# oma219/spumoni

Hardware: AMD Instinct MI355X
Metric: reads/s PML classification, 200 bp reads vs 10-hap human index (higher is better)
Workload: dtype u64

## Files before the change

### spumoni_amd/capi.py

```python
from __future__ import annotations

import ctypes as C
import os
import subprocess
from typing import Optional

import numpy as np

_HERE = os.path.dirname(os.path.abspath(__file__))
LIB_PATH = os.environ.get("SPUMONI_GPU_LIB") or os.path.join(_HERE, "libspumoni_gpu.so")
CSRC = os.path.join(_HERE, "csrc")

SPX_MODE_PML = 0
SPX_MODE_MS = 1

EXPORTS = [
    "spx_last_error",
    "spx_device_count",
    "spx_index_from_runs",
    "spx_index_load_raw",
    "spx_index_free",
    "spx_index_stats",
    "spx_index_device_bytes",
    "spx_index_set_text",
# ... 349 lines not shown
        st = stream if stream is not None else torch.cuda.current_stream(self.device)
        nreads = d_offs.numel() - 1
        cap = int(lib().spx_digest_capacity(kind, k, total_chars))
        if work is None or work[0].numel() < cap or work[1].numel() < nreads + 1:
            work = (torch.empty(cap, dtype=torch.uint8, device=d_seqs.device),
                    torch.empty(nreads + 1, dtype=torch.int64, device=d_seqs.device))
        narrow = any(t is not None and t.element_size() == 2 for t in (d_lengths, d_docs))
        fn = lib().spx_digest_query_batch_device16 if narrow else lib().spx_digest_query_batch_device
        _check(fn(self._h, mode, kind, k, w, _t_ptr(d_seqs), _t_ptr(d_offs), nreads, total_chars, _t_ptr(work[0]), work[0].numel(),
                  _t_ptr(work[1]), _t_ptr(d_lengths), _t_ptr(d_pointers), _t_ptr(d_docs), _t_ptr(d_class), bin_width, max_value_thr,
                  C.c_void_p(st.cuda_stream)))
        return work[1], work

    def digest_query_host(self, mode, kind, k, w, seqs, offs, want_lengths=True, want_docs=False, classify=None):
        seqs = np.ascontiguousarray(seqs, dtype=np.uint8)
        offs = np.ascontiguousarray(offs, dtype=np.uint64)
        nreads = offs.size - 1
        tot = int(offs[-1]) if nreads > 0 else 0
        cap = int(lib().spx_digest_capacity(kind, k, tot))
        out_offs = np.zeros(nreads + 1, dtype=np.uint64)
        lens = np.zeros(cap, dtype=np.uint32) if want_lengths else None
        ptrs = np.zeros(cap, dtype=np.uint64) if mode == SPX_MODE_MS else None
        docs = np.zeros(cap, dtype=np.uint32) if want_docs else None
        cls_ = np.zeros(max(nreads, 1), dtype=CLASS_DTYPE) if classify else None
        bw, thr = classify if classify else (0, 0)
        _check(lib().spx_digest_query_batch(self._h, mode, kind, k, w, _np_ptr(seqs), _np_ptr(offs), nreads,
                                            _np_ptr(out_offs), cap, _np_ptr(lens), _np_ptr(ptrs), _np_ptr(docs),
                                            _np_ptr(cls_), bw, thr))
        dt = int(out_offs[-1])
        out = {"offsets": out_offs}
        if lens is not None:
            out["lengths"] = lens[:dt]
        if ptrs is not None:
            out["pointers"] = ptrs[:dt]
        if docs is not None:
            out["docs"] = docs[:dt]
        if cls_ is not None:
            out["class"] = cls_[:nreads]
        return out

    def votes_device(self, d_lengths, d_docs, d_offs, min_length, d_out=None, stream=None):
        import torch

        L = _spv()
        st = stream if stream is not None else torch.cuda.current_stream(self.device)
        nreads = d_offs.numel() - 1
        if d_lengths.element_size() != d_docs.element_size():
            raise SpxError("d_lengths and d_docs must have the same width")
        if d_out is None:
            d_out = torch.empty((max(nreads, 0), 4), dtype=torch.int32, device=d_offs.device)
        _check(L.spv_votes_device(self._h, _t_ptr(d_lengths), _t_ptr(d_docs), d_lengths.element_size() * 8, _t_ptr(d_offs),
                                  nreads, min(d_lengths.numel(), d_docs.numel()), int(min_length), _t_ptr(d_out),
                                  C.c_void_p(st.cuda_stream)))
        return d_out

    def assign_host(self, mode, seqs, offs, min_length, digest=None):
        from .docvote import VOTE_DTYPE

        L = _spv()
        seqs = np.ascontiguousarray(seqs, dtype=np.uint8)
        offs = np.ascontiguousarray(offs, dtype=np.uint64)
        nreads = offs.size - 1
        kind, k, w = digest if digest else (0, 0, 0)
        rec = np.zeros(max(nreads, 1), dtype=VOTE_DTYPE)
        vals = np.zeros(max(nreads, 1), dtype=np.uint64)
        _check(L.spv_assign_batch(self._h, mode, kind, k, w, _np_ptr(seqs), _np_ptr(offs), nreads, int(min_length),
                                  _np_ptr(rec), _np_ptr(vals)))
        out = np.zeros(nreads, dtype=np.dtype(VOTE_DTYPE.descr + [("values", "<u8")]))
        for f in VOTE_DTYPE.names:
            out[f] = rec[f][:nreads]
        out["values"] = vals[:nreads]
        return out

    def votes_stats(self) -> dict:
        s = SpvVotesStats()
        _check(_spv().spv_last_votes_stats(self._h, C.byref(s)))
        return {f[0]: getattr(s, f[0]) for f in SpvVotesStats._fields_}

    def last_chunk_stats(self) -> dict:
        o = (C.c_uint64 * 4)()
        _check(lib().spx_last_chunk_stats(self._h, C.byref(o)))
        return {"chunk_len": o[0], "chunks_bound": o[1], "rewalked_chars": o[2], "fallback_reads": o[3]}

    def last_stats(self) -> dict:
        s = SpxWalkStats()
        _check(lib().spx_last_walk_stats(self._h, C.byref(s)))
        return {f[0]: getattr(s, f[0]) for f in SpxWalkStats._fields_}


def digester(device: int = 0) -> "Index":
    import torch

    from .synth import RawIndex

    z = torch.zeros(1, dtype=torch.int64)
    return Index.from_raw(RawIndex(heads=torch.zeros(1, dtype=torch.uint8), lens=torch.ones(1, dtype=torch.int64),
                                   thr=z, n=1), device)


def pinned_array(shape, dtype):
    n = int(np.prod(shape)) * np.dtype(dtype).itemsize
    p = lib().spx_host_alloc(max(n, 1))
    if not p:
        raise SpxError(lib().spx_last_error().decode())
    buf = (C.c_char * max(n, 1)).from_address(p)
    arr = np.frombuffer(buf, dtype=dtype, count=int(np.prod(shape))).reshape(shape)

    free = lib().spx_host_free

    class _Owner:
        def __del__(self_inner):
            try:
                free(p)
            except Exception:
                pass

    return arr, _Owner()


def pad_seqs(seqs):
    import torch

    n = seqs.numel()
    padded = torch.zeros(((n + 3) // 4) * 4 + 32, dtype=torch.uint8, device=seqs.device)
    padded[:n] = seqs
    return padded


DOCVOTE_EXPORTS = ["spv_votes_device", "spv_assign_batch", "spv_last_votes_stats"]
_SPV_READY = False


class SpvVotesStats(C.Structure):
    _fields_ = [("reads_short", C.c_uint64), ("reads_medium", C.c_uint64), ("reads_long", C.c_uint64),
                ("reads_empty", C.c_uint64), ("voting_positions", C.c_uint64), ("long_tiles", C.c_uint64),
                ("kernel_ms", C.c_float)]


def _spv() -> C.CDLL:
    global _SPV_READY
    L = lib()
    if not hasattr(L, "spv_assign_batch"):
        raise SpxError(f"{LIB_PATH} has no document votes (spv_assign_batch): there is no CPU fallback")
    if not _SPV_READY:
        vp, u64, u32, i32 = C.c_void_p, C.c_uint64, C.c_uint32, C.c_int
        L.spv_votes_device.argtypes = [vp, vp, vp, i32, vp, u64, u64, u64, vp, vp]
        L.spv_assign_batch.argtypes = [vp, i32, i32, u32, u32, vp, vp, u64, u64, vp, vp]
        L.spv_last_votes_stats.argtypes = [vp, C.POINTER(SpvVotesStats)]
        _SPV_READY = True
    return L


_SPB_READY = False


def _spb() -> C.CDLL:
    global _SPB_READY
    L = lib()
    if not hasattr(L, "spb_build_from_text"):
        raise SpxError(f"{LIB_PATH} has no index builder (spb_build_from_text): there is no CPU fallback for the HIP path")
    if not _SPB_READY:
        vp, u64 = C.c_void_p, C.c_uint64
        L.spb_build_from_text.restype = vp
        L.spb_build_from_text.argtypes = [vp, u64, vp, C.c_uint32, C.c_int, C.c_int]
        L.spb_build_stats.argtypes = [vp, C.POINTER(u64), C.POINTER(u64)]
        L.spb_build_copy.argtypes = [vp, vp, vp, vp, vp, vp, vp, vp]
# ... 85 lines not shown
```

### spumoni_amd/csrc/spx_internal.h

```cpp
#pragma once
#include <hip/hip_runtime.h>

#include <memory>
#include <functional>
#include <mutex>
#include <string>

#include "../../include/spumoni_gpu.h"
#include "spx_layout.h"

namespace spx {

void set_error(const char* fmt, ...);
int hip_fail(hipError_t e, const char* what, const char* file, int line);
int select_device(int device);

#define SPX_HIP(call)                                                        \
    do {                                                                     \
        hipError_t e_ = (call);                                              \
        if (e_ != hipSuccess) return spx::hip_fail(e_, #call, __FILE__, __LINE__); \
    } while (0)

struct QuietOnError {
    hipStream_t st;
    bool device_wide;
    bool ok = false;
    explicit QuietOnError(hipStream_t s, bool wide = false) : st(s), device_wide(wide) {}
    int done(int rc) {
        ok = rc == SPX_OK;
        return rc;
    }
    ~QuietOnError() {
        if (ok) return;
        if (device_wide)
            (void)hipDeviceSynchronize();
        else
            (void)hipStreamSynchronize(st);
    }
};

struct WalkCounters {
    unsigned long long reserved0;
    unsigned long long steps;
    unsigned long long jumps;
    unsigned long long pred_jumps;
    unsigned long long row_loads;
    unsigned long long dir_loads;
    unsigned long long error;
    unsigned long long pad_;
    unsigned long long claim;
};

struct ChunkDesc {
    uint64_t gend;
    uint32_t len;
    uint32_t rd;
};
struct WalkState {
    uint32_t k0;
    uint32_t length;
    uint64_t offp;
    uint64_t sample;
    uint32_t doc;
    uint32_t flags;
};
struct SeamRec {
    uint64_t t;
    uint32_t met;
    uint32_t reset_above;
    WalkState ext;
    uint32_t spec_length, spec_doc;
    uint64_t spec_sample;
};
constexpr uint32_t CKPT_SHIFT = 4;

struct ChunkArgs {
    const ChunkDesc* desc;
    const uint64_t* nchunks;
    WalkState* ends;
    WalkState* ckpt;
    SeamRec* seams;
    uint8_t* flags;
    uint32_t* read_fail;
    const uint64_t* chunk_start;
    WalkState* reentry;
    uint64_t* vtop;
    uint32_t* pending;
    uint32_t round;
    uint32_t last_round;
};
constexpr uint32_t CHUNK_TOP = 0x80000000u, CHUNK_BOTTOM = 0x40000000u, CHUNK_ACTIVE = 0x20000000u;
constexpr uint32_t CHUNK_LEN_MASK = 0x1fffffffu;
constexpr int CHUNK_EXTRA_ROUNDS = 3;

struct BatchArgs {
    const uint8_t* seqs;
    const uint64_t* offs;
    uint64_t nreads;
    uint64_t total_chars;
    uint32_t* out_lengths;
    uint64_t* out_pointers;
    uint32_t* out_docs;
    spx_class* out_class;
    uint64_t bin_width;
    uint64_t bin_magic;
    uint64_t max_value_thr;
    WalkCounters* counters;
    uint32_t lanes_per_wave;
    uint32_t narrow;
    ChunkArgs ch;
    const uint32_t* only_flagged;
    const uint64_t* in_starts;
    uint64_t* len_mask;
    unsigned long long* claim;
    uint64_t len_mask_pairs;
};

}

namespace spx {
struct ArrayOwner {
    int device = 0;
    void* p[10] = {};
    ~ArrayOwner() {
        (void)hipSetDevice(device);
        for (void* a : p)
            if (a) (void)hipFree(a);
    }
};
}

struct spx_index {
    int device = 0;
// ... 147 lines not shown
```

### spumoni_amd/csrc/spx_query.hip

```cpp
#include <algorithm>
#include <chrono>
#include <cstdio>
#include <cstring>
#include <thread>

#include "spx_internal.h"

using namespace spx;

extern "C" {

struct PubSrc {
    const uint64_t* one[4];
    const uint64_t* more;
    int nmore;
};
__global__ void k_publish(uint64_t* dst, PubSrc src) {
    const int t = (int)threadIdx.x;
    if (t < 4) dst[t] = src.one[t] ? *src.one[t] : 0;
    if (t >= 4 && t - 4 < src.nmore) dst[t] = src.more[t - 4];
    __threadfence_system();
}
static int publish(spx_index* ix, const PubSrc& src, hipStream_t st) {
    if (!ix->h_pub) {
        SPX_HIP(hipHostMalloc((void**)&ix->h_pub, 64 * sizeof(uint64_t), hipHostMallocMapped | hipHostMallocCoherent));
        SPX_HIP(hipHostGetDevicePointer((void**)&ix->h_pub_dev, ix->h_pub, 0));
    }
    k_publish<<<1, 64, 0, st>>>(ix->h_pub_dev, src);
    SPX_HIP(hipGetLastError());
    return SPX_OK;
}

uint64_t spx_digest_capacity(int kind, uint32_t k, uint64_t total_chars) {
    const uint64_t body = (kind == SPX_DIGEST_DNA ? (uint64_t)(k ? k : 1) : 1ull) * total_chars;
    return ((body + 3) / 4) * 4 + 32;
}

int spx_digest_batch_device(spx_index* ix, int kind, uint32_t k, uint32_t w, const uint8_t* d_seqs,
                            const uint64_t* d_offsets, uint64_t nreads, uint64_t total_chars,
                            uint8_t* d_out_seqs, uint64_t out_capacity, uint64_t* d_out_offsets, void* stream) {
    if (!ix || !d_seqs || !d_offsets || !d_out_seqs || !d_out_offsets) {
        set_error("null argument");
        return SPX_E_ARG;
    }
    if (((uintptr_t)d_seqs & 15) != 0) {
        set_error("d_seqs must be 16-byte aligned (and readable for round_up(total_chars, 16) + 16 bytes)");
        return SPX_E_ARG;
    }
    if (out_capacity < spx_digest_capacity(kind, k, total_chars)) {
        set_error("d_out_seqs must hold spx_digest_capacity() = %llu bytes",
                  (unsigned long long)spx_digest_capacity(kind, k, total_chars));
        return SPX_E_ARG;
    }
    std::lock_guard<std::mutex> g(ix->mu);
    SPX_HIP(hipSetDevice(ix->device));
    hipStream_t st = (hipStream_t)stream;
    return launch_digest(ix, kind, k, w, d_seqs, d_offsets, nreads, total_chars, d_out_seqs, d_out_offsets, st);
}

static int digest_for_walk(spx_index* ix, int mode, bool ms_lengths, int kind, uint32_t k, uint32_t w, const uint8_t* d_raw,
                           const uint64_t* d_offs, uint64_t nreads, uint64_t total_in, uint8_t* d_dig, uint64_t cap,
                           uint64_t* d_dig_offs, void* stream, const uint64_t** in_starts) {
    *in_starts = nullptr;
    if (!ix || !d_raw || !d_offs || !d_dig || !d_dig_offs) {
        set_error("null argument");
        return SPX_E_ARG;
    }
    if (((uintptr_t)d_raw & 15) != 0) {
        set_error("d_seqs must be 16-byte aligned (and readable for round_up(total_chars, 16) + 16 bytes)");
        return SPX_E_ARG;
    }
    if (cap < spx_digest_capacity(kind, k, total_in)) {
        set_error("the buffer for the digested reads must hold spx_digest_capacity() = %llu bytes",
                  (unsigned long long)spx_digest_capacity(kind, k, total_in));
        return SPX_E_ARG;
    }
    static const bool old_walk = getenv("SPX_OLD_WALK") != nullptr;
    static const int env_parked = getenv("SPX_DIGEST_PARKED") ? atoi(getenv("SPX_DIGEST_PARKED")) : -1;
    const int parked_mode = env_parked >= 0 ? env_parked : ix->digest_parked;
    std::lock_guard<std::mutex> g(ix->mu);
    SPX_HIP(hipSetDevice(ix->device));
    if (ix->num_cus == 0) {
        hipDeviceProp_t prop;
        SPX_HIP(hipGetDeviceProperties(&prop, ix->device));
        ix->num_cus = prop.multiProcessorCount;
    }
    bool park = parked_mode != 1 && ix->rows != nullptr && ix->view.compact && !old_walk && nreads > 0 && nreads < (1ull << 31) &&
                !(mode == SPX_MODE_MS && ms_lengths) && ix->force_lanes_per_wave == 0 &&
                (parked_mode == 2 || nreads * 2 > (uint64_t)ix->num_cus * 20 * 64);
// ... 676 lines not shown
        (void)hipEventRecord(fe[0], st);
    }
    const double t0 = std::chrono::duration<double>(std::chrono::steady_clock::now().time_since_epoch()).count();
    for (int i = 0; i < 3; ++i) {
        if (ix->text_bytes[i] == 0) continue;
        if (text[i]) SPX_HIP(hipMemcpyAsync(text[i], ix->scratch[spx_index::S_TEXT + i].p, ix->text_bytes[i], hipMemcpyDeviceToHost, st));
        if (line_start && line_start[i])
            SPX_HIP(hipMemcpyAsync(line_start[i], ix->scratch[spx_index::S_LINE_START + i].p, (ix->text_nreads + 1) * 8, hipMemcpyDeviceToHost, st));
    }
    if (ix->text_cls_host)
        SPX_HIP(hipMemcpyAsync(ix->text_cls_host, ix->scratch[spx_index::S_CLASS].p, ix->text_nreads * sizeof(spx_class), hipMemcpyDeviceToHost, st));
    if (phase_trace) (void)hipEventRecord(fe[1], st);
    if ((rc = ctx_wait(ix, st)) != SPX_OK) return rc;
    if (phase_trace) {
        float a = 0;
        (void)hipEventElapsedTime(&a, fe[0], fe[1]);
        fprintf(stderr, "[phases] %p fetch: copy out %.3f ms (behind the digits' kernels)\n", (void*)ix, a);
    }
    ix->text_cls_host = nullptr;
    ix->text_ready = false;
    if (timing)
        fprintf(stderr, "[spx] text_fetch: %.2f ms for %.1f MB\n",
                (std::chrono::duration<double>(std::chrono::steady_clock::now().time_since_epoch()).count() - t0) * 1e3,
                (ix->text_bytes[0] + ix->text_bytes[1] + ix->text_bytes[2]) / 1e6);
    return SPX_OK;
}

int spx_query_text_reserve(spx_index* ix, int mode, int digest_kind, uint32_t k, uint64_t max_chars, uint64_t max_reads,
                           uint32_t streams, int with_class, const uint64_t text_bytes[3]) {
    if (!ix || (mode != SPX_MODE_PML && mode != SPX_MODE_MS)) {
        set_error("spx_query_text_reserve: index and a mode");
        return SPX_E_ARG;
    }
    std::lock_guard<std::mutex> hg(ix->host_mu);
    std::lock_guard<std::mutex> g(ix->mu);
    SPX_HIP(hipSetDevice(ix->device));
    hipStream_t st = nullptr;
    int rc;
    if ((rc = ctx_stream_of(ix, &st)) != SPX_OK) return rc;
    const ScratchPlan plan = text_plan(mode, digest_kind, k, max_chars, max_chars, max_reads, streams, with_class != 0, text_bytes, true);
    void* p = nullptr;
    for (int i = 0; i < plan.n; ++i)
        if ((rc = ix->scratch[plan.item[i].slot].reserve(plan.item[i].bytes, &p)) != SPX_OK) return rc;
    const bool need_len = (streams & SPX_TEXT_LENGTHS) || (mode == SPX_MODE_MS && with_class);
    if (mode == SPX_MODE_PML && need_len &&
        (rc = ix->chunk_scr[spx_index::C_LEN_BITS].reserve(len_mask_pairs(max_chars, max_reads) * 16, &p)) != SPX_OK)
        return rc;
    if (!ix->h_pub) {
        PubSrc none{{nullptr, nullptr, nullptr, nullptr}, nullptr, 0};
        if ((rc = publish(ix, none, st)) != SPX_OK) return rc;
    }
    SPX_HIP(hipStreamSynchronize(st));
    return SPX_OK;
}

static int last_counters(spx_index* ix, bool after_ev1, WalkCounters& wc) {
    if (!ix->have_timing) {
        set_error("no query has run on this index yet");
        return SPX_E_ARG;
    }
    SPX_HIP(hipSetDevice(ix->device));
    if (after_ev1) SPX_HIP(hipEventSynchronize(ix->ev1));
    SPX_HIP(hipStreamSynchronize(ix->last_stream));
    SPX_HIP(hipMemcpy(&wc, ix->counters, sizeof wc, hipMemcpyDeviceToHost));
    return SPX_OK;
}

int spx_last_chunk_stats(spx_index* ix, uint64_t out[4]) {
    if (!ix || !out) {
        set_error("null argument");
        return SPX_E_ARG;
    }
    std::lock_guard<std::mutex> g(ix->mu);
    WalkCounters wc;
    const int rc = last_counters(ix, false, wc);
    if (rc != SPX_OK) return rc;
    out[0] = ix->last_chunk_len;
    out[1] = ix->last_chunk_bound;
    out[2] = wc.reserved0;
    out[3] = wc.pad_;
    return SPX_OK;
}

int spx_last_walk_stats(spx_index* ix, spx_walk_stats* out) {
    if (!ix || !out) {
        set_error("null argument");
        return SPX_E_ARG;
    }
    std::lock_guard<std::mutex> g(ix->mu);
    WalkCounters wc;
    const int rc = last_counters(ix, true, wc);
    if (rc != SPX_OK) return rc;
    float ms = 0;
    SPX_HIP(hipEventElapsedTime(&ms, ix->ev0, ix->ev1));
    out->steps = wc.steps;
    out->jumps = wc.jumps;
    out->pred_jumps = wc.pred_jumps;
    out->row_loads = wc.row_loads;
    out->dir_loads = wc.dir_loads;
    out->kernel_ms = ms;
    return walk_error(wc, WALK_ERR_STATS);
}

}
```

### spumoni_amd/csrc/spx_walk_fast.inc

```

enum : uint32_t { Q_LAND = 0, Q_FAT = 1, Q_STEP = 2, Q_READ = 3, Q_CHARS = 4, Q_FATJ = 5, Q_QS = 6, Q_DIR = 7, Q_DONE = 8, Q_SAMP = 9, Q_START = 10, Q_WANT = 11 };
enum : uint32_t {
    F_EMB = 1,
    F_NOROW = 2,
    F_QUIRK = 4,
    F_WIDE = 16,
    F_FADD = 32,
    F_HAVEC = 64,
    F_SAMPD = 128
};
enum : uint32_t { A_STEP = 1, A_EMIT = 2, A_DECIDE = 4 };
#ifndef SPX_STEP_REPS
#define SPX_STEP_REPS 2
#endif
constexpr int STEP_REPS = SPX_STEP_REPS;
constexpr uint32_t OFF_LAST32 = 0xffffffffu;
#ifndef SPX_CHUNK_CLAIM
#define SPX_CHUNK_CLAIM 64
#endif
constexpr uint32_t CHUNK_CLAIM = SPX_CHUNK_CLAIM;
static_assert(CHUNK_CLAIM >= 64, "a claim covers at least one iteration's worst case: 64 lanes ending a read each");

__device__ __forceinline__ uint32_t dpp_swap1(uint32_t v) { return (uint32_t)__builtin_amdgcn_mov_dpp((int)v, 0xB1, 0xf, 0xf, true); }

struct alignas(16) HotLetter {
    uint32_t bmul;
    uint32_t present;
    uint64_t fat0;
};

__device__ __forceinline__ void lf_target_ct(uint32_t LFrun, uint32_t LFoff, uint32_t cums, uint32_t off, uint32_t& k0,
                                             uint32_t& offp, uint32_t& t_out) {
    lf_target_c(LFrun, LFoff, cums, off, k0, offp);
    const uint32_t t = k0 - LFrun;
    t_out = (t < 4 && off <= 126) ? t : 4u;
}

template <int MODE, bool DOC, bool NARROW, int CHUNK = 0, bool EARLY = false, bool DYN = false>
__global__ void __launch_bounds__(WALK_TPB) k_walk_fast(const DevIndex ix, const BatchArgs b) {
    constexpr bool AUX = (MODE == SPX_MODE_MS) || DOC;
    constexpr bool PML = MODE == SPX_MODE_PML;
    if (CHUNK == 2 && b.ch.round > 1 && b.ch.pending[b.ch.round] == 0) return;
    __shared__ HotLetter s_hot[256];
#ifndef SPX_PGRP
#define SPX_PGRP 16
#endif
    constexpr int PGRP = SPX_PGRP, PROW = WALK_TPB + 1;
    constexpr int PLPG = PGRP / 2, PNG = 64 / PLPG;
    __shared__ uint64_t s_ptrs[MODE == SPX_MODE_MS && CHUNK != 2 ? PGRP * PROW : 1];
    constexpr bool DSTAGE = PML && DOC && CHUNK != 2;
    constexpr int DGRP = 32, DROW = DGRP + 2;
    __shared__ uint16_t s_docs[DSTAGE ? WALK_TPB * DROW : 1];
    const LetterInfo* const s_let = ix.letters;
    __shared__ uint32_t s_win[8 * WALK_TPB];
    const char* const rows_b = reinterpret_cast<const char*>(ix.rows);
    const char* const fat_b = reinterpret_cast<const char*>(ix.fat);
    const uint32_t fs = ix.fat_stride;
    const bool lrow = !AUX && fs == 32 && ix.aux == nullptr;
    for (int t = threadIdx.x; t < 256; t += blockDim.x) {
        const LetterInfo li = ix.letters[t];
        s_hot[t] = HotLetter{li.bmul, li.qbeg != li.qend ? 1u : 0u, (uint64_t)(uintptr_t)(fat_b + li.fbase * fs)};
    }
    __syncthreads();
    const char* const dir_b = reinterpret_cast<const char*>(ix.dirrows);
    const char* const fatj_b = reinterpret_cast<const char*>(ix.fat_js);
    const char* const q_b = reinterpret_cast<const char*>(ix.Q);
    const char* const seq_b = reinterpret_cast<const char*>(b.seqs);
    const char* const off_b = reinterpret_cast<const char*>(b.offs);
    const uint32_t R = ix.r;
    const uint32_t fs_shift = fs == 32 ? 5 : 4;
    const bool want_class = PML && CHUNK == 0 && b.out_class != nullptr;
    const bool want_len = PML && CHUNK != 2 && b.out_lengths != nullptr;
    const uint32_t lpw = b.lanes_per_wave;
    const uint32_t nlanes = (uint32_t)((((uint64_t)gridDim.x * blockDim.x) >> 6) * lpw);
    const uint32_t nitems = CHUNK ? (uint32_t)*b.ch.nchunks : (uint32_t)b.nreads;
    const uint64_t ch_org = CHUNK ? b.offs[0] : 0;
    uint8_t* const ch_flags = CHUNK ? b.ch.flags - (ch_org & ~7ull) : nullptr;
    WalkState* const ch_ckpt = CHUNK ? b.ch.ckpt - (ch_org >> CKPT_SHIFT) : nullptr;
    const char* const item_b = CHUNK ? reinterpret_cast<const char*>(b.ch.desc) : off_b;
    constexpr uint32_t ITEM_BYTES = CHUNK ? sizeof(ChunkDesc) : 8;
    const uint32_t tid = threadIdx.x;
    static_assert(!DYN || (CHUNK == 0 && !EARLY), "only the plain, full launch deals its reads on demand");
    uint32_t w_n0 = 0, w_e0 = 0, w_n1 = 0, w_e1 = 0;
    bool w_pend = false;
    bool w_dry = false;
    uint32_t w_wait = DYN ? (uint32_t)((((uint64_t)blockIdx.x * blockDim.x + tid) >> 6) & 31u) + 1u : 0u;
    unsigned long long claimed = 0;

    uint32_t rd = (uint32_t)((((uint64_t)blockIdx.x * blockDim.x + tid) >> 6) * lpw) + (tid & 63);
    uint32_t ph = (rd < nitems && (tid & 63) < lpw) ? Q_READ : Q_DONE;
    const char* addr = ph == Q_READ ? item_b + (uint64_t)rd * ITEM_BYTES : item_b;
    uint32_t seen = 0;
    uint64_t fb = 0;
    uint32_t fl = 0;
    uint32_t c = 0;
    uint64_t base = 0, ibase = 0;
    uint32_t m = 0, x = 0;
    int32_t wi = -1;
    uint64_t q0 = 0, q1 = 0;
    uint32_t k = 0, off = 0;
    uint32_t length = 0;
    uint64_t mbits = 0;
    uint32_t nr = 0;
    uint32_t bin_lo = 0, bin_max = 0, above = 0, below = 0;
    uint64_t sum_max = 0;
    uint64_t sample = 0;
    uint32_t doc = 0;
    uint32_t w_jumps = 0, w_pred = 0, w_rows = 0, w_dir = 0, w_again = 0;
    uint32_t tlimit = 0xffffffffu;
    V16 cka{0, 0, 0, 0}, ckb{0, 0, 0, 0};

#define WIN_AT(w) ((s_win[((uint32_t)(w) >> 2) * WALK_TPB + tid] >> (((uint32_t)(w) & 3) * 8)) & 0xffu)
#define CUR_C c
#define COUNT(var, cond) (var += (uint32_t)__popcll(__builtin_amdgcn_ballot_w64(cond)))

    V16 ga{0, 0, 0, 0}, gb{0, 0, 0, 0};
    uint32_t side_doc = 0;
    Aux side_aux{0, 0};
    uint64_t side_in = 0;
    auto issue_gather = [&]() {
        ga = V16{0, 0, 0, 0};
        gb = V16{0, 0, 0, 0};
#ifndef SPX_PAIR_MIN
#define SPX_PAIR_MIN 24
#endif
        constexpr int pair_min = EARLY ? 65 : SPX_PAIR_MIN;
        if ((int)__popcll(__builtin_amdgcn_ballot_w64(ph != Q_DONE && (fl & F_WIDE))) < pair_min) {
            if (ph != Q_DONE) {
                ga = *reinterpret_cast<const V16*>(addr);
                if (fl & F_WIDE) gb = *reinterpret_cast<const V16*>(addr + 16);
            }
        } else
        {
            typedef uint32_t u32x4 __attribute__((ext_vector_type(4), aligned(4)));
            typedef const __attribute__((address_space(1))) u32x4* GV16;
            const bool odd = tid & 1;
            const bool live = ph != Q_DONE;
            const uint32_t w_own = (live && (fl & F_WIDE)) ? 16u : 0u;
            const uint64_t au = (uint64_t)(uintptr_t)(live ? addr : rows_b);
            const uint64_t pu = u64of(dpp_swap1((uint32_t)au), dpp_swap1((uint32_t)(au >> 32))) + 16;
            const uint32_t w_for = dpp_swap1(w_own);
            const uint64_t a1 = odd ? pu : au, a2 = odd ? au : pu;
            const bool do1 = odd ? w_for != 0 : live, do2 = odd ? live : w_for != 0;
            uint32_t r1x = 0, r1y = 0, r1z = 0, r1w = 0, r2x = 0, r2y = 0, r2z = 0, r2w = 0;
            if (do1) {
                const u32x4 t = *(GV16)(uintptr_t)a1;
                r1x = t.x, r1y = t.y, r1z = t.z, r1w = t.w;
            }
            if (do2) {
                const u32x4 t = *(GV16)(uintptr_t)a2;
                r2x = t.x, r2y = t.y, r2z = t.z, r2w = t.w;
            }
            ga = V16{odd ? r2x : r1x, odd ? r2y : r1y, odd ? r2z : r1z, odd ? r2w : r1w};
            const uint32_t zx = dpp_swap1(odd ? r1x : r2x), zy = dpp_swap1(odd ? r1y : r2y), zz = dpp_swap1(odd ? r1z : r2z),
                           zw = dpp_swap1(odd ? r1w : r2w);
            gb = V16{w_own ? zx : 0u, w_own ? zy : 0u, w_own ? zz : 0u, w_own ? zw : 0u};
        }
        side_doc = 0;
        side_aux = Aux{0, 0};
        side_in = 0;
        claimed = 0;
        if (CHUNK == 0 && b.in_starts != nullptr && ph == Q_READ) side_in = b.in_starts[rd];
        if (DOC && ph == Q_SAMP) side_doc = ix.rundocs[k];
        if (AUX && ph == Q_DIR) side_aux = ix.aux[length];
        if (DYN && w_pend && (tid & 63) == 0) claimed = atomicAdd(b.claim, (unsigned long long)CHUNK_CLAIM);
    };
    if (EARLY) issue_gather();
    while (__builtin_amdgcn_ballot_w64(ph != Q_DONE) != 0) {
        if (!EARLY) issue_gather();
        uint32_t act = 0, hd = 0;
        uint32_t rflag = 0;
        bool pred_ev = false;
        uint32_t d_trun = 0, d_toff = 0, d_srun = 0, d_soff = 0, d_bits = 0;
        Aux d_aux{0, 0};
        bool d_lrow = false;
        uint64_t fbits = 0;
        uint32_t fxi = 0;
        bool flush = false;
        bool pflush = false, pheld = false, pheld_end = false;
        uint32_t pfxi = 0;
        uint64_t phold = 0;
        COUNT(w_rows, ph == Q_LAND);
        COUNT(w_dir, ph == Q_FAT || (ph >= Q_FATJ && ph <= Q_DIR));

        if (ph == Q_LAND) {
            const uint32_t len = ga.x & 0xffffu;
            const uint32_t o = off == OFF_LAST32 ? len - 1 : off;
            if (o >= len) {
                off = o - len;
                k++;
                addr += sizeof(Row32);
            } else {
                off = o;
                q0 = u64of(ga.x, ga.y);
                q1 = u64of(ga.z, ga.w);
                fl = (fl & ~F_NOROW) | F_EMB;
                act = A_STEP;
            }
        } else if (ph == Q_FAT) {
            const uint32_t hq = ga.x;
            const uint32_t w1l = ga.z, w1h = ga.w;
            const bool nosucc = (w1h >> 29) & 1, esc = (w1h >> 30) & 1;
            const bool quirk = fl & F_QUIRK;
            const bool found = nosucc || hq > k || (quirk && hq == k);
            if (found && !esc && !quirk) {
                d_trun = hq - (w1l & 0x7ffffu);
                d_toff = ((w1l >> 20) | (w1h << 12)) & 0xffffu;
                d_srun = ga.y;
                const uint32_t sfield = (w1h >> 4) & 0xffffu;
                const bool ps = (w1h >> 28) & 1;
                d_soff = ps ? sfield : 0u;
                d_bits = ((w1h >> 20) & 0xffu) | ((uint32_t)ps << 8) | ((uint32_t)nosucc << 9) | ((w1h >> 31) << 10) |
                         ((ps ? 0u : (sfield & 0xffu)) << 16);
                if (AUX) d_aux = Aux{u64of(gb.x, gb.y), u64of(gb.z, gb.w)};
                d_lrow = lrow;
                act = A_DECIDE;
            } else if (!found && (w1l & (uint32_t)FAT_SINGLE) && !(fl & F_FADD)) {
                fl |= F_FADD;
                addr += fs;
            } else if (found && esc && !quirk) {
                length = ga.y;
                fl |= F_WIDE;
                ph = Q_DIR;
                addr = dir_b + (uint64_t)length * sizeof(JumpRow);
            } else {
                const uint64_t grp = ((uint64_t)(addr - fat_b) >> fs_shift) >> FJ_SHIFT;
                length = (uint32_t)grp & 3;
                fl &= ~F_WIDE;
                ph = Q_FATJ;
                addr = fatj_b + ((grp * 4) & ~15ull);
            }
        } else if (ph == Q_STEP) {
            act = A_STEP;
        } else if (ph != Q_DONE && ph != Q_SAMP && (!DYN || ph != Q_WANT)) {
            if (ph == Q_READ) {
                if (CHUNK) {
                    m = ga.z & CHUNK_LEN_MASK;
                    base = u64of(ga.x, ga.y) - m;
                    seen = 0;
                    fb = 0;
                    if (CHUNK == 2 && (((ga.z >> 29) & 4) || (b.ch.round > 1 && !((ga.z >> 29) & 1)))) m = 0;
                } else {
                    base = u64of(ga.x, ga.y);
                    m = (uint32_t)(u64of(ga.z, ga.w) - base);
                }
                ibase = (CHUNK == 0 && b.in_starts != nullptr) ? side_in : base;
                if (m == 0) {
                    if (want_class) b.out_class[rd] = spx_class{0, 0, 0};
                    rd += DYN ? 0u : nlanes;
                    ph = DYN ? Q_WANT : (rd < nitems ? Q_READ : Q_DONE);
                    addr = DYN ? rows_b : item_b + (uint64_t)rd * ITEM_BYTES;
                } else {
                    if (NARROW && CHUNK == 0 && m >= 65536) atomicAdd(&b.counters->error, 1ull);
                    x = m;
                    length = 0;
                    sample = ix.init_sample;
                    doc = ix.init_doc;
                    k = ix.init_k;
                    off = (uint32_t)ix.init_off;
                    q0 = ix.init_row.q0;
                    q1 = ix.init_row.q1;
                    fl = 0;
                    wi = -1;
                    mbits = 0;
                    nr = m;
                    if (want_class) {
                        const uint32_t w = (uint32_t)b.bin_width;
                        const uint32_t q = w > 1 ? (uint32_t)__umul64hi((uint64_t)m, b.bin_magic) : m;
                        const uint32_t nb = q > 0 ? q : 1;
                        bin_lo = (nb - 1) * w;
                        bin_max = above = below = 0;
                        sum_max = 0;
                    }
                    act = A_STEP;
                    if (CHUNK == 2) {
                        ph = Q_START;
                        addr = reinterpret_cast<const char*>(b.ch.round > 1 ? b.ch.reentry + rd : b.ch.ends + rd + 1);
                        fl = F_WIDE;
                        act = 0;
                    }
                }
            } else if (ph == Q_CHARS) {
                s_win[0 * WALK_TPB + tid] = ga.x;
                s_win[1 * WALK_TPB + tid] = ga.y;
                s_win[2 * WALK_TPB + tid] = ga.z;
                s_win[3 * WALK_TPB + tid] = ga.w;
                s_win[4 * WALK_TPB + tid] = gb.x;
                s_win[5 * WALK_TPB + tid] = gb.y;
                s_win[6 * WALK_TPB + tid] = gb.z;
                s_win[7 * WALK_TPB + tid] = gb.w;
                ph = Q_STEP;
                act = A_STEP;
            } else if (CHUNK == 2 && ph == Q_START) {
                k = ga.x;
                length = ga.y;
                {
                    const uint64_t offp = u64of(ga.z, ga.w);
                    off = offp == OFF_END ? OFF_LAST32 : (uint32_t)offp;
                }
                sample = u64of(gb.x, gb.y);
                doc = gb.z;
                tlimit = b.ch.round > 1 ? gb.w : 0xffffffffu;
                ph = Q_LAND;
                addr = rows_b + (uint64_t)k * sizeof(Row32);
                fl = F_WIDE;
                {
                    const char* const cp = reinterpret_cast<const char*>(ch_ckpt + ((base + m - 1) >> CKPT_SHIFT));
                    cka = *reinterpret_cast<const V16*>(cp);
                    ckb = *reinterpret_cast<const V16*>(cp + 16);
                }
            } else if (ph == Q_FATJ) {
                const uint32_t lo = (length & 2) ? ga.z : ga.x, hi = (length & 2) ? ga.w : ga.y;
                length = (length & 1) ? hi : lo;
                fl |= F_WIDE;
                ph = Q_QS;
                addr = q_b + (uint64_t)length * 4;
            } else if (ph == Q_QS) {
                const uint32_t e[8] = {ga.x, ga.y, ga.z, ga.w, gb.x, gb.y, gb.z, gb.w};
                const uint32_t room_q = s_let[CUR_C].qend - length;
                uint32_t skip = 0;
#pragma unroll
                for (int t = 0; t < 8; ++t) skip += ((uint32_t)t < room_q && e[t] < k) ? 1u : 0u;
                length += skip;
                if (skip < 8) {
                    ph = Q_DIR;
                    addr = dir_b + (uint64_t)length * sizeof(JumpRow);
                } else {
                    addr = q_b + (uint64_t)length * 4;
                }
            } else {
                JumpRow e;
                e.d0 = u64of(ga.x, ga.y);
                e.d1 = u64of(ga.z, ga.w);
                e.d2 = u64of(gb.x, gb.y);
                e.d3 = u64of(gb.z, gb.w);
                const uint32_t jdir = length;
                const uint32_t qbeg = s_let[CUR_C].qbeg, qend = s_let[CUR_C].qend;
                if (!(fl & F_QUIRK)) {
                    d_trun = jr_THRrun(e);
                    d_toff = (uint32_t)jr_THRoff(e);
                    d_srun = jr_sLFrun(e);
                    d_soff = (uint32_t)jr_sLFoff(e);
                    d_bits = jr_Hs(e) | ((uint32_t)jr_psame(e) << 8) | ((jdir < qend ? 0u : 1u) << 9) | ((jdir <= qbeg ? 1u : 0u) << 10);
                    if (AUX) d_aux = side_aux;
                    act = A_DECIDE;
                } else {
                    const bool has_succ = jdir < qend;
                    const uint32_t trun = jr_THRrun(e);
                    const bool below_thr = !has_succ || (k < trun) || (k == trun && off < (uint32_t)jr_THRoff(e));
                    const uint32_t LFrun_k = (uint32_t)(q0 >> 32), LFoff_k = (uint32_t)(q0 >> 16) & 0xffffu;
                    pred_ev = below_thr;
                    if (AUX) {
                        const Aux a = ix.aux[jdir + ((below_thr && off > 0) ? 1u : 0u)];
                        if (MODE == SPX_MODE_MS) sample = below_thr ? aux_se(a) : aux_ss(a);
                        if (DOC) doc = below_thr ? (aux_docs(a) >> 16) : (aux_docs(a) & 0xffffu);
                    }
                    if (!below_thr) {
                        k = LFrun_k;
                        off = LFoff_k + off;
                    } else if (off > 0) {
                        k = LFrun_k;
                        off = LFoff_k + off - 1;
                    } else {
                        if (jdir <= qbeg) atomicAdd(&b.counters->error, 1ull);
                        const bool ps = jr_psame(e);
                        const uint32_t srun = jr_sLFrun(e);
                        k = ps ? srun : srun - 1;
                        off = ps ? (uint32_t)jr_sLFoff(e) - 1 : OFF_LAST32;
                    }
                    length = 0;
                    fl &= ~(F_EMB | F_QUIRK);
                    rflag = 3;
                    act = A_EMIT;
                }
            }
        }
        if (AUX && ph == Q_SAMP) {
            if (MODE == SPX_MODE_MS) sample = u64of(ga.x, ga.y);
            if (DOC) doc = side_doc & 0xffffu;
            fl |= F_SAMPD;
            ph = Q_STEP;
            act = A_STEP;
        }

        {
            const bool dec = act & A_DECIDE;
            const bool nosucc = (d_bits >> 9) & 1, psame = (d_bits >> 8) & 1;
            const bool below_thr = nosucc || (k < d_trun) || (k == d_trun && off < d_toff);
            COUNT(w_pred, (dec && below_thr) || pred_ev);
            if (dec) {
                if (below_thr && ((d_bits >> 10) & 1)) atomicAdd(&b.counters->error, 1ull);
                const bool last = below_thr && !psame;
                k = d_srun - (last ? 1u : 0u);
                off = last ? OFF_LAST32 : d_soff - (below_thr ? 1u : 0u);
                hd = last ? ((d_bits >> 16) & 0xffu) : (d_bits & 0xffu);
                if (MODE == SPX_MODE_MS) sample = below_thr ? aux_se(d_aux) : aux_ss(d_aux);
                if (DOC) doc = below_thr ? (aux_docs(d_aux) >> 16) : (aux_docs(d_aux) & 0xffffu);
                length = 0;
                fl = (fl & ~(F_EMB | F_QUIRK)) | ((d_lrow && !last) ? F_EMB : 0u);
                rflag = 3;
                act = A_EMIT;
            }
        }

#pragma unroll
        for (int rep = 0; rep < STEP_REPS; ++rep) {
            if (rep > 0 && __builtin_amdgcn_ballot_w64(act != 0) == 0) break;
            bool jumped = false;
            if (act & A_STEP) {
                const bool havec = fl & F_HAVEC;
                if (!havec && wi < 0) {
                    const uint64_t g = ibase + x - 1;
                    const uint64_t end4 = (g + 4) & ~3ull;
                    const uint64_t wbase = end4 >= 32 ? end4 - 32 : 0;
                    wi = (int32_t)(g - wbase);
                    ph = Q_CHARS;
                    addr = seq_b + wbase;
                    fl = (fl | F_WIDE) & ~F_EMB;
                    act = 0;
                } else {
                    const uint32_t cw = WIN_AT(wi < 0 ? 0 : wi);
                    c = havec ? c : cw;
                    wi -= havec ? 0 : 1;
                    const HotLetter hl = s_hot[c];
                    const uint32_t H = (uint32_t)q1 & 0xffu;
                    const bool eq = k < R && H == c;
                    const bool lf = eq && (c < 128 || ((q1 >> 8) & 1));
                    const bool present = hl.present != 0;
                    const bool go_land = eq && (fl & F_NOROW);
                    const bool go_fat = !go_land && present && !lf;
                    const bool go_samp = AUX && !go_land && lf && c >= 128 && !(fl & F_SAMPD);
                    const bool fin = !(go_land || go_fat || go_samp);
                    const bool lfin = fin && present;
                    uint32_t tk, toff, t;
                    lf_target_ct((uint32_t)(q0 >> 32), (uint32_t)(q0 >> 16) & 0xffffu, (uint32_t)(q1 >> 32), off, tk, toff, t);
                    t = lfin ? t : 4u;
                    const char* a_land = rows_b + (uint64_t)k * sizeof(Row32);
                    const char* a_fat = reinterpret_cast<const char*>((uintptr_t)hl.fat0) + (uint64_t)fat_block(k, hl.bmul) * fs;
                    addr = go_land ? a_land : (go_fat ? a_fat : addr);
                    ph = go_land ? Q_LAND : (go_fat ? Q_FAT : ph);
                    if (go_samp) {
                        addr = reinterpret_cast<const char*>(MODE == SPX_MODE_MS ? (const void*)(ix.ss_by_run + k) : (const void*)(ix.rundocs + k));
                        ph = Q_SAMP;
                    }
                    k = lfin ? tk : k;
                    off = lfin ? toff : off;
                    if (fin && !present) {
                        k = s_let[c].frun;
                        off = (uint32_t)s_let[c].foff;
                        if (MODE == SPX_MODE_MS) {
                            sample = 0;
                            if (DOC) doc = ix.doc_at0;
                        }
                    }
                    if (MODE == SPX_MODE_MS) sample -= (lfin && c < 128) ? 1u : 0u;
                    length = (lfin && c < 128) ? length + 1 : (fin ? 0u : length);
                    if (CHUNK) rflag = (lfin && c < 128) ? 0u : (lfin ? 3u : (MODE == SPX_MODE_MS ? 3u : 1u));
                    jumped = go_fat || (lfin && c >= 128);
                    hd = t < 2 ? ((uint32_t)(q1 >> (16 + 8 * t)) & 0xffu) : 0u;
                    uint32_t nf = fl & ~(F_HAVEC | F_SAMPD | (t == 0 ? 0u : F_EMB));
                    nf = go_fat ? ((nf & ~(F_QUIRK | F_FADD | F_WIDE)) | (eq ? F_QUIRK : 0u) | ((AUX || lrow) ? F_WIDE : 0u)) : nf;
                    nf = go_land ? (nf | F_WIDE | F_HAVEC) : nf;
                    nf = go_samp ? ((nf | F_HAVEC) & ~F_WIDE) : nf;
                    fl = nf;
                    act = fin ? A_EMIT : 0u;
                }
            }
            COUNT(w_jumps, jumped);
            if (CHUNK == 2) COUNT(w_again, (act & A_EMIT) != 0);
            if (act & A_EMIT) {
                const uint32_t xi = x - 1;
                x = xi;
                bool met = false;
                if (CHUNK == 2) {
                    const uint64_t gi = base + xi;
                    seen |= rflag;
                    ch_flags[gi] = (uint8_t)rflag;
                    if (PML) {
                        if (NARROW)
                            reinterpret_cast<uint16_t*>(b.out_lengths)[gi] = (uint16_t)length;
                        else
                            b.out_lengths[gi] = length;
                    } else {
                        b.out_pointers[gi] = sample;
                    }
                    if (DOC) {
                        if (NARROW)
                            reinterpret_cast<uint16_t*>(b.out_docs)[gi] = (uint16_t)doc;
                        else
                            b.out_docs[gi] = doc;
                    }
                    const uint64_t my_off = off == OFF_LAST32 ? OFF_END : (uint64_t)off;
                    if (xi != 0 && (gi & ((1u << CKPT_SHIFT) - 1)) == 0) {
                        if (cka.x == k && u64of(cka.z, cka.w) == my_off && xi <= tlimit) {
                            SeamRec sr;
                            sr.t = gi;
                            sr.met = 1 | (b.ch.round << 8);
                            sr.reset_above = seen;
// ... 225 lines not shown
                }
                todo = __builtin_amdgcn_ballot_w64(pflush);
            }
        }
        if (DSTAGE) {
            const uint32_t lane = tid & 63;
            uint64_t todo = __builtin_amdgcn_ballot_w64(pflush);
            while (todo != 0) {
                while (todo != 0) {
                    uint32_t src = 64;
#pragma unroll
                    for (int kx = 0; kx < 8; ++kx) {
                        if (todo != 0) {
                            const uint32_t l = (uint32_t)__builtin_ctzll(todo);
                            todo &= todo - 1;
                            src = (lane >> 3) == (uint32_t)kx ? l : src;
                        }
                    }
                    const bool valid = src < 64;
                    const uint32_t from = valid ? src : lane;
                    const uint32_t sxi = (uint32_t)__shfl((int)pfxi, (int)from);
                    const uint32_t sm = (uint32_t)__shfl((int)m, (int)from);
                    const uint64_t sbase = u64of((uint32_t)__shfl((int)(uint32_t)base, (int)from), (uint32_t)__shfl((int)(uint32_t)(base >> 32), (int)from));
                    const uint32_t e4 = (lane & 7) * 4;
                    const uint64_t lo = sbase + sxi, hi = sbase + sm;
                    const uint64_t p0 = (lo & ~(uint64_t)(DGRP - 1)) + e4;
                    const uint16_t* const sp = &s_docs[((tid & ~63u) + from) * DROW + e4];
                    const uint32_t w0 = *reinterpret_cast<const uint32_t*>(sp), w1 = *reinterpret_cast<const uint32_t*>(sp + 2);
                    if (valid && p0 >= lo && p0 + 4 <= hi) {
                        if (NARROW)
                            *reinterpret_cast<H16x4*>(reinterpret_cast<uint16_t*>(b.out_docs) + p0) = H16x4{u64of(w0, w1)};
                        else
                            *reinterpret_cast<U32x4*>(b.out_docs + p0) = U32x4{w0 & 0xffffu, w0 >> 16, w1 & 0xffffu, w1 >> 16};
                    } else if (valid) {
#pragma unroll
                        for (int t4 = 0; t4 < 4; ++t4) {
                            const uint32_t dv = ((t4 & 2 ? w1 : w0) >> ((t4 & 1) * 16)) & 0xffffu;
                            if (p0 + t4 >= lo && p0 + t4 < hi) {
                                if (NARROW)
                                    reinterpret_cast<uint16_t*>(b.out_docs)[p0 + t4] = (uint16_t)dv;
                                else
                                    b.out_docs[p0 + t4] = dv;
                            }
                        }
                    }
                }
                pflush = false;
                if (pheld) {
                    s_docs[tid * DROW + (DGRP - 1)] = (uint16_t)phold;
                    pheld = false;
                    pflush = pheld_end;
                    pfxi = 0;
                }
                todo = __builtin_amdgcn_ballot_w64(pflush);
            }
        }
        if (PML && want_len) {
            uint64_t todo = __builtin_amdgcn_ballot_w64(flush);
            const uint32_t lane = tid & 63;
            while (todo != 0) {
                const uint32_t l = (uint32_t)__builtin_ctzll(todo);
                todo &= todo - 1;
                const uint64_t wbits = u64of((uint32_t)__builtin_amdgcn_readlane((int)(uint32_t)fbits, l),
                                             (uint32_t)__builtin_amdgcn_readlane((int)(uint32_t)(fbits >> 32), l));
                const uint32_t wxi = (uint32_t)__builtin_amdgcn_readlane((int)fxi, l);
                const uint32_t wnr = (uint32_t)__builtin_amdgcn_readlane((int)nr, l);
                const uint32_t wm = (uint32_t)__builtin_amdgcn_readlane((int)m, l);
                const uint64_t wbase = u64of((uint32_t)__builtin_amdgcn_readlane((int)(uint32_t)base, l),
                                             (uint32_t)__builtin_amdgcn_readlane((int)(uint32_t)(base >> 32), l));
                const uint32_t cnt = wm - wxi;
                const uint64_t t = wbits >> lane;
                const uint32_t v = t != 0 ? (uint32_t)__builtin_ctzll(t) : wnr - (wxi + lane);
                if (lane < cnt) {
                    if (NARROW)
                        reinterpret_cast<uint16_t*>(b.out_lengths)[wbase + wxi + lane] = (uint16_t)v;
                    else
                        b.out_lengths[wbase + wxi + lane] = v;
                }
            }
        }
        if (PML && CHUNK != 2 && flush) nr = fbits != 0 ? fxi + (uint32_t)__builtin_ctzll(fbits) : nr;
    }
#undef WIN_AT
#undef CUR_C
#undef COUNT
    if ((tid & 63) == 0) {
        if (CHUNK == 2) {
            atomicAdd(&b.counters->reserved0, (unsigned long long)w_again);
        } else {
            atomicAdd(&b.counters->jumps, (unsigned long long)w_jumps);
            atomicAdd(&b.counters->pred_jumps, (unsigned long long)w_pred);
        }
        atomicAdd(&b.counters->row_loads, (unsigned long long)w_rows);
        atomicAdd(&b.counters->dir_loads, (unsigned long long)w_dir);
    }
    (void)sample;
    (void)doc;
    (void)s_ptrs;
    (void)s_docs;
    (void)seen;
    (void)fb;
    (void)ch_flags;
    (void)ch_ckpt;
    (void)tlimit;
    (void)cka;
    (void)ckb;
    (void)w_again;
    (void)w_n0, (void)w_e0, (void)w_n1, (void)w_e1, (void)w_pend, (void)w_dry, (void)w_wait, (void)claimed;
    if (CHUNK != 2 && blockIdx.x == 0 && tid == 0) atomicAdd(&b.counters->steps, (unsigned long long)(b.offs[b.nreads] - b.offs[0]));
}
```

Baseline: 1.095 billion.

## Double-buffer read character window and prefetch next window during other phases

Doubles the per-thread shared-memory character window to two halves. When a lane's window is nearly exhausted, it issues the load for the next 32 bytes of the read alongside the other side loads. On exhaustion it flips halves instead of entering a dedicated Q_CHARS load phase, removing a stall iteration per window. It also adds an iteration counter with a new diagnostic API, at the cost of an extra ballot/popcount and an atomic per wave. The change doubles s_win LDS use, which may reduce occupancy, and adds register pressure from the prefetch buffers.

```diff
diff --git a/include/spumoni_walkdiag.h b/include/spumoni_walkdiag.h
--- /dev/null
+++ b/include/spumoni_walkdiag.h
@@ -0,0 +1,13 @@
+#ifndef SPUMONI_WALKDIAG_H
+#define SPUMONI_WALKDIAG_H
+#include "spumoni_gpu.h"
+#ifdef __cplusplus
+extern "C" {
+#endif
+
+int spx_last_walk_iterations(spx_index *ix, uint64_t *out);
+
+#ifdef __cplusplus
+}
+#endif
+#endif
diff --git a/spumoni_amd/capi.py b/spumoni_amd/capi.py
--- a/spumoni_amd/capi.py
+++ b/spumoni_amd/capi.py
@@ -455,6 +455,13 @@
         _check(lib().spx_last_chunk_stats(self._h, C.byref(o)))
         return {"chunk_len": o[0], "chunks_bound": o[1], "rewalked_chars": o[2], "fallback_reads": o[3]}
 
+    def last_lane_iterations(self) -> int:
+        f = lib().spx_last_walk_iterations
+        f.argtypes = [C.c_void_p, C.POINTER(C.c_uint64)]
+        o = C.c_uint64(0)
+        _check(f(self._h, C.byref(o)))
+        return int(o.value)
+
     def last_stats(self) -> dict:
         s = SpxWalkStats()
         _check(lib().spx_last_walk_stats(self._h, C.byref(s)))
diff --git a/spumoni_amd/csrc/spx_internal.h b/spumoni_amd/csrc/spx_internal.h
--- a/spumoni_amd/csrc/spx_internal.h
+++ b/spumoni_amd/csrc/spx_internal.h
@@ -49,6 +49,7 @@
     unsigned long long error;
     unsigned long long pad_;
     unsigned long long claim;
+    unsigned long long iterations;
 };
 
 struct ChunkDesc {
diff --git a/spumoni_amd/csrc/spx_query.hip b/spumoni_amd/csrc/spx_query.hip
--- a/spumoni_amd/csrc/spx_query.hip
+++ b/spumoni_amd/csrc/spx_query.hip
@@ -5,6 +5,7 @@
 #include <thread>
 
 #include "spx_internal.h"
+#include "../../include/spumoni_walkdiag.h"
 
 using namespace spx;
 
@@ -847,6 +848,19 @@
     return SPX_OK;
 }
 
+int spx_last_walk_iterations(spx_index* ix, uint64_t* out) {
+    if (!ix || !out) {
+        set_error("null argument");
+        return SPX_E_ARG;
+    }
+    std::lock_guard<std::mutex> g(ix->mu);
+    WalkCounters wc;
+    const int rc = last_counters(ix, false, wc);
+    if (rc != SPX_OK) return rc;
+    *out = wc.iterations;
+    return SPX_OK;
+}
+
 int spx_last_walk_stats(spx_index* ix, spx_walk_stats* out) {
     if (!ix || !out) {
         set_error("null argument");
diff --git a/spumoni_amd/csrc/spx_walk_fast.inc b/spumoni_amd/csrc/spx_walk_fast.inc
--- a/spumoni_amd/csrc/spx_walk_fast.inc
+++ b/spumoni_amd/csrc/spx_walk_fast.inc
@@ -7,7 +7,9 @@
     F_WIDE = 16,
     F_FADD = 32,
     F_HAVEC = 64,
-    F_SAMPD = 128
+    F_SAMPD = 128,
+    F_NEXTW = 256,
+    F_WHALF = 512
 };
 enum : uint32_t { A_STEP = 1, A_EMIT = 2, A_DECIDE = 4 };
 #ifndef SPX_STEP_REPS
@@ -52,7 +54,7 @@
     constexpr int DGRP = 32, DROW = DGRP + 2;
     __shared__ uint16_t s_docs[DSTAGE ? WALK_TPB * DROW : 1];
     const LetterInfo* const s_let = ix.letters;
-    __shared__ uint32_t s_win[8 * WALK_TPB];
+    __shared__ uint32_t s_win[16 * WALK_TPB];
     const char* const rows_b = reinterpret_cast<const char*>(ix.rows);
     const char* const fat_b = reinterpret_cast<const char*>(ix.fat);
     const uint32_t fs = ix.fat_stride;
@@ -97,6 +99,7 @@
     uint64_t base = 0, ibase = 0;
     uint32_t m = 0, x = 0;
     int32_t wi = -1;
+    uint32_t wrem = 0;
     uint64_t q0 = 0, q1 = 0;
     uint32_t k = 0, off = 0;
     uint32_t length = 0;
@@ -106,11 +109,13 @@
     uint64_t sum_max = 0;
     uint64_t sample = 0;
     uint32_t doc = 0;
-    uint32_t w_jumps = 0, w_pred = 0, w_rows = 0, w_dir = 0, w_again = 0;
+    uint32_t w_jumps = 0, w_pred = 0, w_rows = 0, w_dir = 0, w_again = 0, w_iters = 0;
     uint32_t tlimit = 0xffffffffu;
     V16 cka{0, 0, 0, 0}, ckb{0, 0, 0, 0};
 
-#define WIN_AT(w) ((s_win[((uint32_t)(w) >> 2) * WALK_TPB + tid] >> (((uint32_t)(w) & 3) * 8)) & 0xffu)
+    static_assert(8u * WALK_TPB == (F_WHALF << 2), "WIN_HALF is the flag bit shifted into place");
+#define WIN_HALF ((fl & F_WHALF) << 2)
+#define WIN_AT(w) ((s_win[WIN_HALF + ((uint32_t)(w) >> 2) * WALK_TPB + tid] >> (((uint32_t)(w) & 3) * 8)) & 0xffu)
 #define CUR_C c
 #define COUNT(var, cond) (var += (uint32_t)__popcll(__builtin_amdgcn_ballot_w64(cond)))
 
@@ -118,6 +123,8 @@
     uint32_t side_doc = 0;
     Aux side_aux{0, 0};
     uint64_t side_in = 0;
+    V16 side_wa{0, 0, 0, 0}, side_wb{0, 0, 0, 0};
+    bool side_w = false;
     auto issue_gather = [&]() {
         ga = V16{0, 0, 0, 0};
         gb = V16{0, 0, 0, 0};
@@ -160,6 +167,13 @@
         side_aux = Aux{0, 0};
         side_in = 0;
         claimed = 0;
+        side_w = (ph <= Q_STEP || (ph >= Q_FATJ && ph <= Q_DIR) || ph == Q_SAMP) && wi < STEP_REPS && wrem != 0 && !(fl & F_NEXTW);
+        if (side_w) {
+            const uint64_t wb = ibase + wrem;
+            const char* const wp = seq_b + (wb >= 32 ? wb - 32 : 0);
+            side_wa = *reinterpret_cast<const V16*>(wp);
+            side_wb = *reinterpret_cast<const V16*>(wp + 16);
+        }
         if (CHUNK == 0 && b.in_starts != nullptr && ph == Q_READ) side_in = b.in_starts[rd];
         if (DOC && ph == Q_SAMP) side_doc = ix.rundocs[k];
         if (AUX && ph == Q_DIR) side_aux = ix.aux[length];
@@ -182,6 +196,19 @@
         uint64_t phold = 0;
         COUNT(w_rows, ph == Q_LAND);
         COUNT(w_dir, ph == Q_FAT || (ph >= Q_FATJ && ph <= Q_DIR));
+        COUNT(w_iters, ph != Q_DONE);
+        if (side_w) {
+            const uint32_t oh = WIN_HALF ^ (8u * WALK_TPB);
+            s_win[oh + 0 * WALK_TPB + tid] = side_wa.x;
+            s_win[oh + 1 * WALK_TPB + tid] = side_wa.y;
+            s_win[oh + 2 * WALK_TPB + tid] = side_wa.z;
+            s_win[oh + 3 * WALK_TPB + tid] = side_wa.w;
+            s_win[oh + 4 * WALK_TPB + tid] = side_wb.x;
+            s_win[oh + 5 * WALK_TPB + tid] = side_wb.y;
+            s_win[oh + 6 * WALK_TPB + tid] = side_wb.z;
+            s_win[oh + 7 * WALK_TPB + tid] = side_wb.w;
+            fl |= F_NEXTW;
+        }
 
         if (ph == Q_LAND) {
             const uint32_t len = ga.x & 0xffffu;
@@ -262,6 +289,7 @@
                     q1 = ix.init_row.q1;
                     fl = 0;
                     wi = -1;
+                    wrem = 0;
                     mbits = 0;
                     nr = m;
                     if (want_class) {
@@ -281,14 +309,15 @@
                     }
                 }
             } else if (ph == Q_CHARS) {
-                s_win[0 * WALK_TPB + tid] = ga.x;
-                s_win[1 * WALK_TPB + tid] = ga.y;
-                s_win[2 * WALK_TPB + tid] = ga.z;
-                s_win[3 * WALK_TPB + tid] = ga.w;
-                s_win[4 * WALK_TPB + tid] = gb.x;
-                s_win[5 * WALK_TPB + tid] = gb.y;
-                s_win[6 * WALK_TPB + tid] = gb.z;
-                s_win[7 * WALK_TPB + tid] = gb.w;
+                const uint32_t wh = WIN_HALF;
+                s_win[wh + 0 * WALK_TPB + tid] = ga.x;
+                s_win[wh + 1 * WALK_TPB + tid] = ga.y;
+                s_win[wh + 2 * WALK_TPB + tid] = ga.z;
+                s_win[wh + 3 * WALK_TPB + tid] = ga.w;
+                s_win[wh + 4 * WALK_TPB + tid] = gb.x;
+                s_win[wh + 5 * WALK_TPB + tid] = gb.y;
+                s_win[wh + 6 * WALK_TPB + tid] = gb.z;
+                s_win[wh + 7 * WALK_TPB + tid] = gb.w;
                 ph = Q_STEP;
                 act = A_STEP;
             } else if (CHUNK == 2 && ph == Q_START) {
@@ -409,11 +438,18 @@
             bool jumped = false;
             if (act & A_STEP) {
                 const bool havec = fl & F_HAVEC;
+                if (!havec && wi < 0 && (fl & F_NEXTW)) {
+                    const uint64_t wb = ibase + wrem;
+                    wi = wb >= 32 ? 31 : (int32_t)wb - 1;
+                    wrem = wrem >= 32 ? wrem - 32 : 0u;
+                    fl = (fl ^ F_WHALF) & ~F_NEXTW;
+                }
                 if (!havec && wi < 0) {
                     const uint64_t g = ibase + x - 1;
                     const uint64_t end4 = (g + 4) & ~3ull;
                     const uint64_t wbase = end4 >= 32 ? end4 - 32 : 0;
                     wi = (int32_t)(g - wbase);
+                    wrem = wbase > ibase ? (uint32_t)(wbase - ibase) : 0u;
                     ph = Q_CHARS;
                     addr = seq_b + wbase;
                     fl = (fl | F_WIDE) & ~F_EMB;
@@ -805,6 +841,7 @@
         if (PML && CHUNK != 2 && flush) nr = fbits != 0 ? fxi + (uint32_t)__builtin_ctzll(fbits) : nr;
     }
 #undef WIN_AT
+#undef WIN_HALF
 #undef CUR_C
 #undef COUNT
     if ((tid & 63) == 0) {
@@ -816,6 +853,7 @@
         }
         atomicAdd(&b.counters->row_loads, (unsigned long long)w_rows);
         atomicAdd(&b.counters->dir_loads, (unsigned long long)w_dir);
+        atomicAdd(&b.counters->iterations, (unsigned long long)w_iters);
     }
     (void)sample;
     (void)doc;
```

New measurement: 1.053 billion. 0.962x the previous value.
